# MahdiGhafoorian/NLML_HPE

Hardware: AMD Instinct MI355X
Metric: faces_per_sec (higher is better)
Workload: dtype f16x2s

## Files before the change

nlml_hpe_amd/csrc/abi.cpp:

```cpp
#include <hip/hip_runtime_api.h>

#include <cstdio>
#include <cstdlib>
#include <cstring>

#include "../../include/nlml_hpe.h"
#include "abi_internal.h"
#include "centroid_ref.h"
#include "layout.h"
#include "powell.h"

namespace nlml {
static thread_local char g_err[256] = "";
int fail(int code, const char* msg) {
  std::snprintf(g_err, sizeof g_err, "%s", msg ? msg : "unknown error");
  return code ? code : NLML_E_BADARG;
}
int hip_launch_status() {
  const hipError_t e = hipGetLastError();
  return e == hipSuccess ? 0 : fail((int)e, hipGetErrorString(e));
}
}

using namespace nlml;

static bool known_mode(int mode) { return mode == NLML_MODE_F32 || mode == NLML_MODE_BF16 || mode == NLML_MODE_F16X2 || mode == NLML_MODE_F16X2S; }
static bool split_f16(int mode) { return mode == NLML_MODE_F16X2 || mode == NLML_MODE_F16X2S; }

extern "C" {

int nlml_abi_version(void) { return NLML_ABI_VERSION; }
const char* nlml_last_error(void) { return g_err; }

int nlml_normalize_ipd(const float* raw, int64_t B, int normalize, float* out, uint8_t* valid, void* stream) {
  if (B < 0 || (B > 0 && (!raw || !out))) return fail(NLML_E_BADARG, "normalize_ipd: null buffer or negative B");
  if ((reinterpret_cast<uintptr_t>(raw) | reinterpret_cast<uintptr_t>(out)) & 15)
    return fail(NLML_E_BADARG, "normalize_ipd: raw/out must be 16-byte aligned");
  return launch_normalize_ipd(raw, B, normalize, out, valid, stream);
}

int nlml_normalize_centroid(const float* raw, int64_t B, float* out, uint8_t* valid, double* stats, void* stream) {
  if (B < 0 || (B > 0 && (!raw || !out))) return fail(NLML_E_BADARG, "normalize_centroid: null buffer or negative B");
  if ((reinterpret_cast<uintptr_t>(raw) | reinterpret_cast<uintptr_t>(out)) & 15)
    return fail(NLML_E_BADARG, "normalize_centroid: raw/out must be 16-byte aligned");
  if (reinterpret_cast<uintptr_t>(stats) & 7) return fail(NLML_E_BADARG, "normalize_centroid: stats must be 8-byte aligned");
  return launch_normalize_centroid(raw, B, out, valid, stats, stream);
}

int nlml_normalize_centroid_host(const float* h_raw, int64_t B, float* h_out, uint8_t* h_valid, double* h_stats) {
  if (B < 0 || (B > 0 && (!h_raw || !h_out))) return fail(NLML_E_BADARG, "normalize_centroid_host: null buffer or negative B");
  for (int64_t b = 0; b < B; ++b) {
    const int v = cn_face_host(h_raw + b * NLML_F_REFERENCE, h_out + b * NLML_F_REFERENCE, h_stats ? h_stats + 4 * b : nullptr);
    if (h_valid) h_valid[b] = (uint8_t)v;
  }
  return 0;
}

size_t nlml_encoder_heads_packed_bytes(int F, int mode) {
  if (F <= 0 || !known_mode(mode)) return 0;
  return blob_bytes_for(F, mode);
}

int nlml_encoder_heads_pack(int F, int mode, const float* const h_enc_w[6], const float* const h_enc_b[6],
                            const float* const h_head_w[3][5], const float* const h_head_b[3][5], void* h_blob,
                            size_t blob_bytes) {
  if (!known_mode(mode)) return fail(NLML_E_BADARG, "pack: unsupported mode");
  if (!h_enc_w || !h_enc_b || !h_head_w || !h_head_b) return fail(NLML_E_BADARG, "pack: null table");
  return pack_blob(F, mode, h_enc_w, h_enc_b, h_head_w, h_head_b, h_blob, blob_bytes);
}

static int check_blob_args(int64_t B, int F, const void* blob, size_t blob_bytes, const float* out, int* mode) {
  if (B < 0 || F <= 0) return fail(NLML_E_BADARG, "encoder_heads: negative B or bad F");
  if (B > 0 && (!blob || !out)) return fail(NLML_E_BADARG, "encoder_heads: null buffer");
  if (reinterpret_cast<uintptr_t>(blob) & 15) return fail(NLML_E_BADARG, "encoder_heads: blob must be 16-byte aligned");
  if (blob_bytes == blob_bytes_for(F, NLML_MODE_F32)) *mode = NLML_MODE_F32;
  else if (blob_bytes == blob_bytes_for(F, NLML_MODE_BF16)) *mode = NLML_MODE_BF16;
  else if (blob_bytes == blob_bytes_for(F, NLML_MODE_F16X2)) *mode = NLML_MODE_F16X2;
  else if (blob_bytes == blob_bytes_for(F, NLML_MODE_F16X2S)) *mode = NLML_MODE_F16X2S;
  else return fail(NLML_E_BADBLOB, "encoder_heads: blob size does not match F in any mode");
  return 0;
}

static const int64_t kSmallMax = 4096;
static int64_t streamed_min() {
  static const int64_t v = [] { const char* e = getenv("NLML_K2_STREAMED_MIN"); return e && e[0] ? (int64_t)atoll(e) : (int64_t)-1; }();
  return v;
}

enum K2Form { K2_FUSED, K2_SMALL, K2_STREAMED, K2_AUTO };

static int k2_forward(K2Form form, bool landmarks, const float* x, int64_t ldx, const float* raw, int normalize, int64_t B, int F,
                      const void* blob, size_t blob_bytes, float* out, float* latent, uint8_t* valid, void* workspace, size_t ws_bytes,
                      void* stream) {
  const char* no_input = nullptr;
  if (B > 0 && landmarks && !raw) no_input = "landmarks_to_pose: null raw";
  if (B > 0 && !landmarks && (!x || ldx < F)) no_input = "encoder_heads: null x or ldx < F";
  if (no_input && form == K2_AUTO && landmarks) return fail(NLML_E_BADARG, no_input);
  int mode = 0;
  if (int rc = check_blob_args(B, F, blob, blob_bytes, out, &mode)) return rc;
  if (form == K2_SMALL && !split_f16(mode)) return fail(NLML_E_BADARG, "small-batch path: NLML_MODE_F16X2 / NLML_MODE_F16X2S blob only");
  if (form == K2_STREAMED && mode != NLML_MODE_F16X2S) return fail(NLML_E_BADARG, "streamed-tail path: NLML_MODE_F16X2S blob only");
  if (no_input) return fail(NLML_E_BADARG, no_input);
  const int split = mode == NLML_MODE_F16X2S;
  if (form == K2_AUTO) {
    if (split_f16(mode) && B <= kSmallMax) form = K2_SMALL;
    else if (split && streamed_min() >= 0 && B >= streamed_min() && k2_input(x, ldx, raw, normalize, F).vec4) form = K2_STREAMED;
    else form = K2_FUSED;
  }
  if (form == K2_SMALL)
    return launch_encoder_heads_f16x2_small(x, ldx, raw, normalize, B, F, blob, out, latent, valid, workspace, ws_bytes, split, stream);
  if (form == K2_STREAMED)
    return launch_encoder_heads_f16x2_tailws(x, ldx, raw, normalize, B, F, blob, out, latent, valid, workspace, ws_bytes, stream);
  if (mode == NLML_MODE_BF16) return launch_encoder_heads_bf16(x, ldx, raw, normalize, B, F, blob, out, latent, valid, stream);
  if (split_f16(mode)) return launch_encoder_heads_f16x2(x, ldx, raw, normalize, B, F, blob, out, latent, valid, split, stream);
  return launch_encoder_heads_f32(x, ldx, raw, normalize, B, F, blob, out, latent, valid, nullptr, nullptr, stream);
}

int nlml_encoder_heads_fwd(const float* x, int64_t ldx, int64_t B, int F, const void* blob, size_t blob_bytes,
                           float* out, float* latent, uint8_t* valid, void* stream) {
  return k2_forward(K2_FUSED, false, x, ldx, nullptr, 0, B, F, blob, blob_bytes, out, latent, valid, nullptr, 0, stream);
}

int nlml_encoder_heads_fwd_debug(const float* x, int64_t ldx, int64_t B, int F, const void* blob, size_t blob_bytes,
                                 float* out, float* latent, float* pre_tanh, unsigned long long* stamps, void* stream) {
  int mode = 0;
  if (int rc = check_blob_args(B, F, blob, blob_bytes, out, &mode)) return rc;
  if (mode != NLML_MODE_F32) return fail(NLML_E_BADARG, "debug build: f32 blob only");
  if (B > 0 && (!x || ldx < F)) return fail(NLML_E_BADARG, "encoder_heads: null x or ldx < F");
  return launch_encoder_heads_f32(x, ldx, nullptr, 0, B, F, blob, out, latent, nullptr, pre_tanh, stamps, stream);
}

int nlml_landmarks_to_pose(const float* raw, int64_t B, int normalize, const void* blob, size_t blob_bytes,
                           float* out, float* latent, uint8_t* valid, void* stream) {
  return k2_forward(K2_FUSED, true, nullptr, 0, raw, normalize, B, NLML_F_REFERENCE, blob, blob_bytes, out, latent, valid, nullptr, 0, stream);
}

size_t nlml_encoder_heads_small_workspace_bytes(int64_t B, int F) { return small_workspace_bytes(B, F); }

int nlml_encoder_heads_fwd_small(const float* x, int64_t ldx, int64_t B, int F, const void* blob, size_t blob_bytes,
                                 float* out, float* latent, uint8_t* valid, void* workspace, size_t ws_bytes, void* stream) {
  return k2_forward(K2_SMALL, false, x, ldx, nullptr, 0, B, F, blob, blob_bytes, out, latent, valid, workspace, ws_bytes, stream);
}

int nlml_landmarks_to_pose_small(const float* raw, int64_t B, int normalize, const void* blob, size_t blob_bytes,
                                 float* out, float* latent, uint8_t* valid, void* workspace, size_t ws_bytes, void* stream) {
  return k2_forward(K2_SMALL, true, nullptr, 0, raw, normalize, B, NLML_F_REFERENCE, blob, blob_bytes, out, latent, valid, workspace, ws_bytes, stream);
}

int nlml_encoder_heads_fwd_streamed(const float* x, int64_t ldx, int64_t B, int F, const void* blob, size_t blob_bytes,
                                    float* out, float* latent, uint8_t* valid, void* workspace, size_t ws_bytes, void* stream) {
  return k2_forward(K2_STREAMED, false, x, ldx, nullptr, 0, B, F, blob, blob_bytes, out, latent, valid, workspace, ws_bytes, stream);
}

int nlml_landmarks_to_pose_streamed(const float* raw, int64_t B, int normalize, const void* blob, size_t blob_bytes,
                                    float* out, float* latent, uint8_t* valid, void* workspace, size_t ws_bytes, void* stream) {
  return k2_forward(K2_STREAMED, true, nullptr, 0, raw, normalize, B, NLML_F_REFERENCE, blob, blob_bytes, out, latent, valid, workspace, ws_bytes, stream);
}

size_t nlml_encoder_heads_workspace_bytes(int64_t B, int F) {
  const size_t a = small_workspace_bytes(B, F), b = tailws_workspace_bytes(B, F);
  return a > b ? a : b;
}

int nlml_encoder_heads_fwd_ws(const float* x, int64_t ldx, int64_t B, int F, const void* blob, size_t blob_bytes,
                              float* out, float* latent, uint8_t* valid, void* workspace, size_t ws_bytes, void* stream) {
  return k2_forward(K2_AUTO, false, x, ldx, nullptr, 0, B, F, blob, blob_bytes, out, latent, valid, workspace, ws_bytes, stream);
}

int nlml_landmarks_to_pose_ws(const float* raw, int64_t B, int normalize, const void* blob, size_t blob_bytes,
                              float* out, float* latent, uint8_t* valid, void* workspace, size_t ws_bytes, void* stream) {
  return k2_forward(K2_AUTO, true, nullptr, 0, raw, normalize, B, NLML_F_REFERENCE, blob, blob_bytes, out, latent, valid, workspace, ws_bytes, stream);
}

static int check_td_fast_alignment(const float* Wm, const float* x, int64_t ldx, const char* who) {
  if ((reinterpret_cast<uintptr_t>(Wm) & 15) || (reinterpret_cast<uintptr_t>(x) & 15) || (ldx & 3)) {
    static thread_local char msg[160];
    snprintf(msg, sizeof msg, "%s: NLML_TD_ORDER_FAST needs Wm and x 16-byte aligned and ldx %% 4 == 0", who);
    return fail(NLML_E_BADARG, msg);
  }
  return 0;
}

int nlml_tucker_objective_ex(const float* Wm, const float* x, int64_t ldx, const int32_t* x_index,
                             const double* params, const double* cos_params, int64_t N, double* err, double* x_hat,
                             int order, void* stream) {
  if (order != NLML_TD_ORDER_FAST && order != NLML_TD_ORDER_REFERENCE) return fail(NLML_E_BADARG, "tucker_objective: unknown order");
  if (N < 0) return fail(NLML_E_BADARG, "tucker_objective: negative N");
  if (N > 0 && (!Wm || !x || !params || !cos_params || !err)) return fail(NLML_E_BADARG, "tucker_objective: null buffer");
  if (N > 0 && ldx < NLML_F_REFERENCE) return fail(NLML_E_BADARG, "tucker_objective: ldx < 1404");
  if (N > 0 && order == NLML_TD_ORDER_FAST)
    if (int rc = check_td_fast_alignment(Wm, x, ldx, "tucker_objective")) return rc;
  return launch_tucker_objective(Wm, x, ldx, x_index, params, cos_params, N, err, x_hat, order, stream);
}

int nlml_tucker_objective(const float* Wm, const float* x, int64_t ldx, const int32_t* x_index,
                          const double* params, const double* cos_params, int64_t N, double* err, double* x_hat,
                          void* stream) {
  return nlml_tucker_objective_ex(Wm, x, ldx, x_index, params, cos_params, N, err, x_hat, NLML_TD_ORDER_REFERENCE, stream);
}

int nlml_video_post_ex(const float* pose_rad, const float* raw, const uint8_t* valid, int64_t S, double frame_w,
                       double frame_h, double alpha, double max_jump, double size, double* state, double* smoothed,
                       double* centre, double* endpoints, uint8_t* updated, void* stream) {
  if (S < 0) return fail(NLML_E_BADARG, "video_post: negative S");
  if (S > 0 && (!pose_rad || !raw || !state || !smoothed || !centre || !endpoints))
    return fail(NLML_E_BADARG, "video_post: null buffer");
  return launch_video_post(pose_rad, raw, valid, S, frame_w, frame_h, alpha, max_jump, size, state, smoothed, centre,
                           endpoints, updated, stream);
}

int nlml_video_post(const float* pose_rad, const float* raw, const uint8_t* valid, int64_t S, double frame_w,
                    double frame_h, double alpha, double max_jump, double size, double* state, double* smoothed,
                    double* centre, double* endpoints, void* stream) {
  return nlml_video_post_ex(pose_rad, raw, valid, S, frame_w, frame_h, alpha, max_jump, size, state, smoothed, centre, endpoints,
                            nullptr, stream);
}

int nlml_cosine_table(const float* angles_rad, int64_t n, const double* cos_params, int R, double* out, void* stream) {
  if (n < 0 || R < 0) return fail(NLML_E_BADARG, "cosine_table: negative size");
  if (n > 0 && R > 0 && (!angles_rad || !cos_params || !out)) return fail(NLML_E_BADARG, "cosine_table: null buffer");
  return launch_cosine_table(angles_rad, n, cos_params, R, out, stream);
}

int nlml_mode5_product(const float* core, const float* U_feat, int Q, int R5, int M, float* W, void* stream) {
  if (Q < 0 || R5 < 0 || M < 0) return fail(NLML_E_BADARG, "mode5_product: negative size");
  if (Q > 0 && M > 0 && (!W || (R5 > 0 && (!core || !U_feat)))) return fail(NLML_E_BADARG, "mode5_product: null buffer");
  return launch_mode5_product(core, U_feat, Q, R5, M, W, stream);
}

static bool eval_k_ok(int K) { return K >= 0 && K <= NLML_POSE_EVAL_MAX_INTERVALS; }
static int64_t eval_records(int64_t B) { return (B + NLML_POSE_EVAL_FACES_PER_RECORD - 1) / NLML_POSE_EVAL_FACES_PER_RECORD; }

size_t nlml_pose_eval_record_len(int n_intervals) { return eval_k_ok(n_intervals) ? (size_t)(12 + 2 * n_intervals) : 0; }
size_t nlml_pose_eval_result_len(int n_intervals) { return eval_k_ok(n_intervals) ? (size_t)(14 + 2 * n_intervals) : 0; }
size_t nlml_pose_eval_workspace_bytes(int64_t B, int n_intervals) {
  if (B < 0 || !eval_k_ok(n_intervals)) return 0;
  return (size_t)eval_records(B) * nlml_pose_eval_record_len(n_intervals) * sizeof(double);
}

static bool misaligned8(const void* p) { return (reinterpret_cast<uintptr_t>(p) & 7) != 0; }

int nlml_pose_eval(const float* pose_rad, const double* pred_deg, const uint8_t* valid, const double* gt_deg, int64_t B,
                   const double* h_lo, const double* h_hi, int decimals, const double* h_intervals, const int32_t* h_axes,
                   int n_intervals, void* workspace, size_t workspace_bytes, double* record_out, double* result_out,
                   double* pred_out, uint8_t* keep_out, void* stream) {
  if (B < 0) return fail(NLML_E_BADARG, "pose_eval: negative B");
  if ((pose_rad && pred_deg) || (B > 0 && !pose_rad && !pred_deg))
    return fail(NLML_E_BADARG, "pose_eval: give exactly one of pose_rad and pred_deg");
  if (B > 0 && !gt_deg) return fail(NLML_E_BADARG, "pose_eval: null gt_deg");
  if (!h_lo || !h_hi || !result_out) return fail(NLML_E_BADARG, "pose_eval: null lo / hi / result_out");
  if (!eval_k_ok(n_intervals)) return fail(NLML_E_BADARG, "pose_eval: number of intervals outside [0, NLML_POSE_EVAL_MAX_INTERVALS]");
  if (n_intervals > 0 && (!h_intervals || !h_axes)) return fail(NLML_E_BADARG, "pose_eval: null intervals / axes");
  if (decimals > 15) return fail(NLML_E_BADARG, "pose_eval: decimals > 15");
  const size_t need = nlml_pose_eval_workspace_bytes(B, n_intervals);
  if (workspace_bytes < need || (need > 0 && !workspace)) return fail(NLML_E_BADARG, "pose_eval: workspace too small");
  if (misaligned8(pred_deg) || misaligned8(gt_deg) || misaligned8(workspace) || misaligned8(record_out) || misaligned8(result_out) ||
      misaligned8(pred_out) || (reinterpret_cast<uintptr_t>(pose_rad) & 3))
    return fail(NLML_E_BADARG, "pose_eval: f64 buffers must be 8-byte aligned, pose_rad 4-byte aligned");
  PoseEvalArgs a{};
  for (int i = 0; i < 3; ++i) { a.lo[i] = h_lo[i]; a.hi[i] = h_hi[i]; }
  for (int k = 0; k < n_intervals; ++k) {
    if (h_axes[k] < 0 || h_axes[k] > 2) return fail(NLML_E_BADARG, "pose_eval: interval axis outside {0, 1, 2}");
    a.axes[k] = h_axes[k];
    a.ivl[k][0] = h_intervals[2 * k];
    a.ivl[k][1] = h_intervals[2 * k + 1];
  }
  a.scale = 1.0;
  for (int i = 0; i < decimals; ++i) a.scale *= 10.0;
  a.K = n_intervals;
  a.decimals = decimals;
  return launch_pose_eval(pose_rad, pred_deg, valid, gt_deg, B, a, static_cast<double*>(workspace), record_out, result_out, pred_out,
                          keep_out, stream);
}

int nlml_pose_eval_merge(const double* records, int64_t n, int n_intervals, double* record_out, double* result_out, void* stream) {
  if (n < 0) return fail(NLML_E_BADARG, "pose_eval_merge: negative record count");
  if (!eval_k_ok(n_intervals)) return fail(NLML_E_BADARG, "pose_eval_merge: number of intervals outside [0, NLML_POSE_EVAL_MAX_INTERVALS]");
  if ((n > 0 && !records) || !result_out) return fail(NLML_E_BADARG, "pose_eval_merge: null records / result_out");
  if (misaligned8(records) || misaligned8(record_out) || misaligned8(result_out))
    return fail(NLML_E_BADARG, "pose_eval_merge: buffers must be 8-byte aligned");
  return launch_pose_eval_merge(records, n, n_intervals, record_out, result_out, stream);
}

size_t nlml_powell_state_bytes(void) { return sizeof(PowellState); }

int nlml_powell_init(void* h_state, const double* h_x0, double xtol, double ftol) {
  if (!h_state || !h_x0) return fail(NLML_E_BADARG, "powell_init: null pointer");
  powell_init(*static_cast<PowellState*>(h_state), h_x0, xtol, ftol);
  return 0;
}

int nlml_powell_step(void* h_state, double fin, double* h_xeval) {
  if (!h_state || !h_xeval) return fail(NLML_E_BADARG, "powell_step: null pointer");
  PowellState& s = *static_cast<PowellState*>(h_state);
  const bool need = powell_step(s, fin);
  if (need) std::memcpy(h_xeval, s.xeval, sizeof s.xeval);
  return need ? 1 : 0;
}

int nlml_powell_result(const void* h_state, double* h_x, double* h_fval, int* h_nfev, int* h_nit, int* h_status) {
  if (!h_state || !h_x) return fail(NLML_E_BADARG, "powell_result: null pointer");
  const PowellState& s = *static_cast<const PowellState*>(h_state);
  std::memcpy(h_x, s.x, sizeof s.x);
  if (h_fval) *h_fval = s.fval;
  if (h_nfev) *h_nfev = s.nfev;
  if (h_nit) *h_nit = s.iter;
  if (h_status) *h_status = s.status;
  return 0;
}

int nlml_tucker_powell_ex(const float* Wm, const float* x, int64_t ldx, const double* cos_params, int64_t N,
                          const double* x0, double* result, double* fval, int32_t* nfev, int32_t* nit,
                          int32_t* status, int order, void* stream) {
  if (order != NLML_TD_ORDER_FAST && order != NLML_TD_ORDER_REFERENCE) return fail(NLML_E_BADARG, "tucker_powell: unknown order");
  if (N < 0) return fail(NLML_E_BADARG, "tucker_powell: negative N");
  if (N > 0 && (!Wm || !x || !cos_params || !result)) return fail(NLML_E_BADARG, "tucker_powell: null buffer");
  if (N > 0 && ldx < NLML_F_REFERENCE) return fail(NLML_E_BADARG, "tucker_powell: ldx < 1404");
  if (N > 0 && order == NLML_TD_ORDER_FAST)
    if (int rc = check_td_fast_alignment(Wm, x, ldx, "tucker_powell")) return rc;
  return launch_tucker_powell(Wm, x, ldx, cos_params, N, x0, result, fval, nfev, nit, status, order, stream);
}

int nlml_tucker_powell(const float* Wm, const float* x, int64_t ldx, const double* cos_params, int64_t N,
                       const double* x0, double* result, double* fval, int32_t* nfev, int32_t* nit,
                       int32_t* status, void* stream) {
  return nlml_tucker_powell_ex(Wm, x, ldx, cos_params, N, x0, result, fval, nfev, nit, status, NLML_TD_ORDER_REFERENCE, stream);
}

static_assert(PW_NMAX == 3 + NLML_TUCKER_RANK_MAX && PW_N == 3 + 5, "powell.h's state sizes follow the ranks");
static bool rank_ok(int r_id) { return r_id >= NLML_TUCKER_RANK_MIN && r_id <= NLML_TUCKER_RANK_MAX; }
static int bad_rank(const char* who, int r_id) {
  static thread_local char msg[160];
  snprintf(msg, sizeof msg, "%s: identity rank %d outside [%d, %d]", who, r_id, NLML_TUCKER_RANK_MIN, NLML_TUCKER_RANK_MAX);
  return fail(NLML_E_SHAPE, msg);
}

int nlml_tucker_objective_r(const float* Wm, const float* x, int64_t ldx, const int32_t* x_index, const double* params,
                            const double* cos_params, int64_t N, double* err, double* x_hat, int r_id, int order, void* stream) {
  if (!rank_ok(r_id)) return bad_rank("tucker_objective_r", r_id);
  if (r_id == 5) return nlml_tucker_objective_ex(Wm, x, ldx, x_index, params, cos_params, N, err, x_hat, order, stream);
  if (order != NLML_TD_ORDER_FAST && order != NLML_TD_ORDER_REFERENCE) return fail(NLML_E_BADARG, "tucker_objective_r: unknown order");
  if (N < 0) return fail(NLML_E_BADARG, "tucker_objective_r: negative N");
  if (N > 0 && (!Wm || !x || !params || !cos_params || !err)) return fail(NLML_E_BADARG, "tucker_objective_r: null buffer");
  if (N > 0 && ldx < NLML_F_REFERENCE) return fail(NLML_E_BADARG, "tucker_objective_r: ldx < 1404");
  if (N > 0 && order == NLML_TD_ORDER_FAST)
    if (int rc = check_td_fast_alignment(Wm, x, ldx, "tucker_objective_r")) return rc;
  return launch_tucker_objective_r(Wm, x, ldx, x_index, params, cos_params, N, err, x_hat, r_id, order, stream);
}

int nlml_tucker_powell_r(const float* Wm, const float* x, int64_t ldx, const double* cos_params, int64_t N, const double* x0,
                         double* result, double* fval, int32_t* nfev, int32_t* nit, int32_t* status, int r_id, int order,
                         void* stream) {
  if (!rank_ok(r_id)) return bad_rank("tucker_powell_r", r_id);
  if (r_id == 5) return nlml_tucker_powell_ex(Wm, x, ldx, cos_params, N, x0, result, fval, nfev, nit, status, order, stream);
  if (order != NLML_TD_ORDER_FAST && order != NLML_TD_ORDER_REFERENCE) return fail(NLML_E_BADARG, "tucker_powell_r: unknown order");
  if (N < 0) return fail(NLML_E_BADARG, "tucker_powell_r: negative N");
  if (N > 0 && (!Wm || !x || !cos_params || !result)) return fail(NLML_E_BADARG, "tucker_powell_r: null buffer");
  if (N > 0 && ldx < NLML_F_REFERENCE) return fail(NLML_E_BADARG, "tucker_powell_r: ldx < 1404");
  if (N > 0 && order == NLML_TD_ORDER_FAST)
    if (int rc = check_td_fast_alignment(Wm, x, ldx, "tucker_powell_r")) return rc;
  return launch_tucker_powell_r(Wm, x, ldx, cos_params, N, x0, result, fval, nfev, nit, status, r_id, order, stream);
}

static bool dim_ok(int n) { return n >= 3 + NLML_TUCKER_RANK_MIN && n <= 3 + NLML_TUCKER_RANK_MAX; }

size_t nlml_powell_state_bytes_n(int n) { return dim_ok(n) ? sizeof(PowellStateN) : 0; }

int nlml_powell_init_n(void* h_state, int n, const double* h_x0, double xtol, double ftol) {
  if (!dim_ok(n)) return bad_rank("powell_init_n", n - 3);
  if (!h_state || !h_x0) return fail(NLML_E_BADARG, "powell_init_n: null pointer");
  PowellStateN& s = *static_cast<PowellStateN*>(h_state);
  std::memset(h_state, 0, sizeof(PowellStateN));
  s.set_dim(n);
  powell_init(s, h_x0, xtol, ftol);
  return 0;
}

int nlml_powell_step_n(void* h_state, double fin, double* h_xeval) {
  if (!h_state || !h_xeval) return fail(NLML_E_BADARG, "powell_step_n: null pointer");
  PowellStateN& s = *static_cast<PowellStateN*>(h_state);
  if (!dim_ok(s.n)) return bad_rank("powell_step_n", s.n - 3);
  const bool need = powell_step(s, fin);
  if (need) std::memcpy(h_xeval, s.xeval, sizeof(double) * s.n);
  return need ? 1 : 0;
}

int nlml_powell_result_n(const void* h_state, double* h_x, double* h_fval, int* h_nfev, int* h_nit, int* h_status) {
  if (!h_state || !h_x) return fail(NLML_E_BADARG, "powell_result_n: null pointer");
  const PowellStateN& s = *static_cast<const PowellStateN*>(h_state);
  if (!dim_ok(s.n)) return bad_rank("powell_result_n", s.n - 3);
  std::memcpy(h_x, s.x, sizeof(double) * s.n);
  if (h_fval) *h_fval = s.fval;
  if (h_nfev) *h_nfev = s.nfev;
  if (h_nit) *h_nit = s.iter;
  if (h_status) *h_status = s.status;
  return 0;
}

}
```

nlml_hpe_amd/csrc/encoder_heads_f16x2_tailws.hip:

```cpp
#include <hip/hip_runtime.h>

#include "../../include/nlml_hpe.h"
#include "abi_internal.h"
#include "encoder_heads_f16x2_dev.h"
#include "layout.h"

#if defined(__HIP_DEVICE_COMPILE__) && !defined(__gfx950__)
#error "global_load_lds_dwordx4: gfx950"
#endif

namespace nlml {
namespace hx {

typedef unsigned u4 __attribute__((ext_vector_type(4)));
#ifdef TW_NO_PRIO
#define TW_PRIO(p) do { } while (0)
#else
#define TW_PRIO(p) __builtin_amdgcn_s_setprio(p)
#endif
typedef __attribute__((address_space(3))) const char LdsC;
typedef __attribute__((address_space(3))) char LdsW;

struct TwArgs {
  const void* blob;
  const u4* h3;
  float* out;
  float* latent;
  int64_t B, nfb;
};

constexpr int TW_SLOT = 65536;
constexpr int tw_bias_n16(int s) { return kStages[s].jobs * kStages[s].nb * 8; }
constexpr int tw_bias_off(int s) {
  int o = 0;
  for (int t = ST_E3; t < s; ++t) o += tw_bias_n16(t) * 16;
  return o;
}
constexpr int TW_O_BIAS = 2 * TW_SLOT;
constexpr int TW_O_LAT = TW_O_BIAS + ((tw_bias_off(NUM_STAGES) + 511) / 512) * 512;
constexpr int TW_LAT_WAVE = 3 * 2 * 256;
constexpr int TW_LDS = TW_O_LAT + 8 * TW_LAT_WAVE;
static_assert(TW_LDS <= 163840, "LDS map");

constexpr int TW_HEAD_UNITS = 9, TW_UNITS = 4 + 3 * TW_HEAD_UNITS;
__device__ __forceinline__ void tw_unit(const HdrRegs& H, int idx, uint32_t& off, uint32_t& n16) {
  constexpr uint32_t J3 = stage_job_w16_const(ST_E3), J4 = stage_job_w16_const(ST_E4), J5 = stage_job_w16_const(ST_E5);
  constexpr uint32_t K0 = stage_job_w16_const(ST_H0), K1 = stage_job_w16_const(ST_H1), K2 = stage_job_w16_const(ST_H2);
  constexpr uint32_t K3 = stage_job_w16_const(ST_H3), K4 = stage_job_w16_const(ST_H4);
  static_assert(2 * J3 * 16 == TW_SLOT && 2 * J4 * 16 <= TW_SLOT && J5 * 16 <= TW_SLOT && 4 * K0 * 16 <= TW_SLOT && K1 * 16 <= TW_SLOT &&
                    2 * K2 * 16 == TW_SLOT && 2 * K3 * 16 <= TW_SLOT && K4 * 16 <= TW_SLOT,
                "a unit fits a buffer");
  if (idx < 2) { n16 = 2 * J3; off = H.w_off(ST_E3) + idx * 2 * J3; }
  else if (idx == 2) { n16 = 2 * J4; off = H.w_off(ST_E4); }
  else if (idx == 3) { n16 = J5; off = H.w_off(ST_E5); }
  else {
    const int k = idx - 4, g = k / TW_HEAD_UNITS, r = k - TW_HEAD_UNITS * g;
    if (r == 0) { n16 = 4 * K0; off = H.w_off(ST_H0) + 4 * g * K0; }
    else if (r <= 4) { n16 = K1; off = H.w_off(ST_H1) + (4 * g + (r - 1)) * K1; }
    else if (r <= 6) { n16 = 2 * K2; off = H.w_off(ST_H2) + (4 * g + 2 * (r - 5)) * K2; }
    else if (r == 7) { n16 = 2 * K3; off = H.w_off(ST_H3) + 2 * g * K3; }
    else { n16 = K4; off = H.w_off(ST_H4) + g * K4; }
  }
}

template <int K16, int NCH = 2>
__device__ __forceinline__ void tw_job2(f32x16 (&acc)[2], LdsC* w0, LdsC* w1, int wstep, LdsC* b0, LdsC* b1, const h8 (&in)[K16][2]) {
  typedef const __attribute__((address_space(3))) h8 LdsH8;
#pragma unroll
  for (int c = 0; c < NCH; ++c)
#pragma unroll
    for (int q = 0; q < 4; ++q) {
      const f32x4 v = *reinterpret_cast<const __attribute__((address_space(3))) f32x4*>((c ? b1 : b0) + q * 16);
      acc[c][4 * q + 0] = v[0];
      acc[c][4 * q + 1] = v[1];
      acc[c][4 * q + 2] = v[2];
      acc[c][4 * q + 3] = v[3];
    }
  TW_PRIO(2);
#pragma unroll
  for (int ks = 0; ks < K16; ++ks) {
    h8 wf[NCH][2];
#pragma unroll
    for (int c = 0; c < NCH; ++c)
#pragma unroll
      for (int p = 0; p < 2; ++p) wf[c][p] = *reinterpret_cast<LdsH8*>((c ? w1 : w0) + ks * wstep + p * 1024);
#pragma unroll
    for (int t = 0; t < 3; ++t)
#pragma unroll
      for (int c = 0; c < NCH; ++c)
        acc[c] = __builtin_amdgcn_mfma_f32_32x32x16_f16(wf[c][t == 0 ? 1 : 0], in[ks][t == 1 ? 1 : 0], acc[c], 0, 0, 0);
  }
  TW_PRIO(0);
}

template <int K16>
__device__ __forceinline__ void tw_job2p(f32x16 (&acc)[2], LdsC* w0, LdsC* w1, int wstep, LdsC* b0, LdsC* b1, const h8 (&in)[K16][2]) {
  typedef const __attribute__((address_space(3))) h8 LdsH8;
#pragma unroll
  for (int c = 0; c < 2; ++c)
#pragma unroll
    for (int q = 0; q < 4; ++q) {
      const f32x4 v = *reinterpret_cast<const __attribute__((address_space(3))) f32x4*>((c ? b1 : b0) + q * 16);
      acc[c][4 * q + 0] = v[0];
      acc[c][4 * q + 1] = v[1];
      acc[c][4 * q + 2] = v[2];
      acc[c][4 * q + 3] = v[3];
    }
  h8 wf[2][2][2];
#pragma unroll
  for (int c = 0; c < 2; ++c)
#pragma unroll
    for (int p = 0; p < 2; ++p) wf[0][c][p] = *reinterpret_cast<LdsH8*>((c ? w1 : w0) + p * 1024);
  TW_PRIO(2);
  __builtin_amdgcn_sched_barrier(0);
#pragma unroll
  for (int ks = 0; ks < K16; ++ks) {
#pragma unroll
    for (int m = 0; m < 6; ++m) {
      const int t = m >> 1, c = m & 1;
      acc[c] = __builtin_amdgcn_mfma_f32_32x32x16_f16(wf[ks & 1][c][t == 0 ? 1 : 0], in[ks][t == 1 ? 1 : 0], acc[c], 0, 0, 0);
      __builtin_amdgcn_sched_barrier(0);
      if (m < 4 && ks + 1 < K16)
        wf[(ks + 1) & 1][m & 1][m < 2 ? 1 : 0] = *reinterpret_cast<LdsH8*>(((m & 1) ? w1 : w0) + (ks + 1) * wstep + (m < 2 ? 1024 : 0));
      __builtin_amdgcn_sched_barrier(0);
    }
  }
  TW_PRIO(0);
}

__global__ __launch_bounds__(512) void tail_ws_kernel(TwArgs a) {
  __shared__ __attribute__((aligned(1024))) char lds[TW_LDS];
  const int tid = threadIdx.x, lane = tid & 63, f = lane & 31, h = lane >> 5;
  const int wv = __builtin_amdgcn_readfirstlane(tid >> 6);
  const HdrRegs H = load_hdr(reinterpret_cast<const Header*>(a.blob));
  const h8* const blob8 = reinterpret_cast<const h8*>(a.blob);
  const f32x4* const blob4 = reinterpret_cast<const f32x4*>(a.blob);

  int64_t fbg = (int64_t)blockIdx.x * 8 + wv;
  const bool wave_live = fbg < a.nfb;
  fbg = wave_live ? fbg : a.nfb - 1;
  const int64_t row = fbg * 32 + f;
  const bool row_live = wave_live && row < a.B;

  LdsW* const ring = (LdsW*)(lds);
  auto issue = [&](int idx, int slot_off) {
    if (idx >= TW_UNITS) return;
    uint32_t off, n16;
    tw_unit(H, idx, off, n16);
    const int npieces = (int)(n16 >> 6);
#pragma unroll
    for (int i = 0; i < TW_SLOT / 8192; ++i) {
      const int pc = wv + 8 * i;
      if (pc < npieces)
        __builtin_amdgcn_global_load_lds((const __attribute__((address_space(1))) void*)(blob8 + off + pc * 64 + lane),
                                         (__attribute__((address_space(3))) void*)(ring + slot_off + pc * 1024), 16, 0, 0);
    }
  };
#ifdef TW_STAMPS
  int tw_u = 0;
#define TWS(i)                                                                                                                \
  do {                                                                                                                        \
    if (a.latent && lane == 0)                                                                                                \
      reinterpret_cast<unsigned long long*>(a.latent)[((size_t)blockIdx.x * 8 + wv) * 96 + (i)] = __builtin_amdgcn_s_memtime(); \
  } while (0)
#define TW_STAMP_MID() TWS(2 + 2 * tw_u)
#define TW_STAMP_END() do { TWS(3 + 2 * tw_u); ++tw_u; } while (0)
#else
#define TWS(i) do { } while (0)
#define TW_STAMP_MID() do { } while (0)
#define TW_STAMP_END() do { } while (0)
#endif
  TWS(0);
  issue(0, 0);

  {
    f32x4* const bl = reinterpret_cast<f32x4*>(lds + TW_O_BIAS);
#pragma unroll
    for (int s = ST_E3; s < NUM_STAGES; ++s) {
      const f32x4* src = blob4 + H.b_off(s);
      for (int i = tid; i < tw_bias_n16(s); i += 512) bl[tw_bias_off(s) / 16 + i] = src[i];
    }
  }
  h8 x3[16][2];
  {
    const u4* src = a.h3 + (size_t)fbg * (16 * 2 * 64) + lane;
#pragma unroll
    for (int ks = 0; ks < 16; ++ks)
#pragma unroll
      for (int p = 0; p < 2; ++p) x3[ks][p] = __builtin_bit_cast(h8, src[(ks * 2 + p) * 64]);
  }
  asm volatile("s_waitcnt vmcnt(0)" ::: "memory");
  __syncthreads();
  TWS(1);

  int cur = 0;
  LdsC* const bias0 = (LdsC*)(lds + TW_O_BIAS) + 64 * h;
  LdsC* const wl0 = (LdsC*)(lds) + lane * 16;
  LdsW* const latw = (LdsW*)(lds + TW_O_LAT) + wv * TW_LAT_WAVE + f * 8;
#ifdef TW_NO_SKEW
  const bool late = false;
#else
  const bool late = wv >= 4;
#endif
#define TW_BEGIN(idx) issue((idx) + 1, cur ^ TW_SLOT); LdsC* const wl = wl0 + cur
#define TW_MID()                                      \
  TW_STAMP_MID();                                     \
  asm volatile("s_waitcnt vmcnt(0)" ::: "memory");    \
  if (late) __syncthreads()
#define TW_END()                                      \
  asm volatile("s_waitcnt vmcnt(0)" ::: "memory");    \
  if (!late) __syncthreads();                         \
  TW_STAMP_END();                                     \
  cur ^= TW_SLOT

  f32x16 acc[2];
  auto emit = [&](auto act, const f32x16& ac, float inv, h8 (&d0)[2], h8 (&d1)[2]) {
    h8 fr[2][2];
    frags_from_acc<decltype(act)::value>(ac, inv, fr);
    d0[0] = fr[0][0]; d0[1] = fr[0][1]; d1[0] = fr[1][0]; d1[1] = fr[1][1];
  };
  constexpr std::integral_constant<int, ACT_RELU> RELU{};
  constexpr std::integral_constant<int, ACT_TANH> TANH{};
  const float inv3 = H.inv_scale[ST_E3], inv4 = H.inv_scale[ST_E4], inv5 = H.inv_scale[ST_E5];
  constexpr int JB3 = (int)(stage_job_w16_const(ST_E3) * 16), JB4 = (int)(stage_job_w16_const(ST_E4) * 16);

  h8 x4[8][2];
#pragma unroll
  for (int u = 0; u < 2; ++u) {
    TW_BEGIN(u);
    LdsC* const b = bias0 + tw_bias_off(ST_E3) + (2 * u) * 128;
    tw_job2p<16>(acc, wl, wl + JB3, 2048, b, b + 128, x3);
    TW_MID();
    emit(RELU, acc[0], inv3, x4[4 * u], x4[4 * u + 1]);
    emit(RELU, acc[1], inv3, x4[4 * u + 2], x4[4 * u + 3]);
    TW_END();
  }
  h8 x5[4][2];
  {
    TW_BEGIN(2);
    LdsC* const b = bias0 + tw_bias_off(ST_E4);
    tw_job2<8>(acc, wl, wl + JB4, 2048, b, b + 128, x4);
    TW_MID();
    emit(TANH, acc[0], inv4, x5[0], x5[1]);
    emit(TANH, acc[1], inv4, x5[2], x5[3]);
    TW_END();
  }
  {
    TW_BEGIN(3);
    LdsC* const b = bias0 + tw_bias_off(ST_E5);
    tw_job2<4>(acc, wl, wl + 2048, 4096, b, b + 128, x5);
    TW_MID();
#ifndef TW_STAMPS
    if (a.latent && row_live) {
#pragma unroll
      for (int nb = 0; nb < 2; ++nb)
#pragma unroll
        for (int q = 0; q < 16; ++q) {
          const int rowi = 32 * nb + (q & 3) + 8 * (q >> 2) + 4 * h, g = rowi >> 4, cc = rowi & 15;
          if (g < 3 && cc < 3) a.latent[row * NLML_LATENT + 3 * g + cc] = acc[nb][q] * inv5;
        }
    }
#endif
#pragma unroll
    for (int nb = 0; nb < 2; ++nb) {
      h8 fr[2][2];
      frags_from_acc<ACT_NONE>(acc[nb], inv5, fr);
#pragma unroll
      for (int p = 0; p < 2; ++p)
#pragma unroll
        for (int pc = 0; pc < 2; ++pc)
          if (2 * nb + p < 3 && h == 0) {
            const u4 t = __builtin_bit_cast(u4, fr[p][pc]);
            typedef unsigned u2 __attribute__((ext_vector_type(2)));
            *reinterpret_cast<__attribute__((address_space(3))) u2*>(latw + ((2 * nb + p) * 2 + pc) * 256) = u2{t[0], t[1]};
          }
    }
    TW_END();
  }
#pragma unroll 1
  for (int g = 0; g < 3; ++g) {
    const int u0 = 4 + TW_HEAD_UNITS * g;
    const float i0 = H.inv_scale[ST_H0], i1 = H.inv_scale[ST_H1], i2 = H.inv_scale[ST_H2], i3 = H.inv_scale[ST_H3];
    h8 xa[8][2];
    {
      TW_BEGIN(u0);
      h8 xin[1][2];
#pragma unroll
      for (int pc = 0; pc < 2; ++pc) {
        typedef unsigned u2 __attribute__((ext_vector_type(2)));
        const u2 t = *reinterpret_cast<const __attribute__((address_space(3))) u2*>((LdsC*)latw + (g * 2 + pc) * 256);
        xin[0][pc] = __builtin_bit_cast(h8, u4{h == 0 ? t[0] : 0u, h == 0 ? t[1] : 0u, 0u, 0u});
      }
      LdsC* const b = bias0 + tw_bias_off(ST_H0) + (4 * g) * 128;
      constexpr int JB = (int)(stage_job_w16_const(ST_H0) * 16);
#pragma unroll
      for (int jj = 0; jj < 2; ++jj) {
        tw_job2<1>(acc, wl + (2 * jj) * JB, wl + (2 * jj + 1) * JB, 2048, b + (2 * jj) * 128, b + (2 * jj + 1) * 128, xin);
        if (jj == 1) { TW_MID(); }
        emit(RELU, acc[0], i0, xa[4 * jj], xa[4 * jj + 1]);
        emit(RELU, acc[1], i0, xa[4 * jj + 2], xa[4 * jj + 3]);
      }
      TW_END();
    }
    h8 xb[16][2];
#pragma unroll
    for (int j = 0; j < 4; ++j) {
      TW_BEGIN(u0 + 1 + j);
      LdsC* const b = bias0 + tw_bias_off(ST_H1) + (4 * g + j) * 256;
      tw_job2p<8>(acc, wl, wl + 2048, 4096, b, b + 128, xa);
      TW_MID();
      emit(RELU, acc[0], i1, xb[4 * j], xb[4 * j + 1]);
      emit(RELU, acc[1], i1, xb[4 * j + 2], xb[4 * j + 3]);
      TW_END();
    }
    h8 xc[8][2];
#pragma unroll
    for (int u = 0; u < 2; ++u) {
      TW_BEGIN(u0 + 5 + u);
      constexpr int JB = (int)(stage_job_w16_const(ST_H2) * 16);
      LdsC* const b = bias0 + tw_bias_off(ST_H2) + (4 * g + 2 * u) * 128;
      tw_job2p<16>(acc, wl, wl + JB, 2048, b, b + 128, xb);
      TW_MID();
      emit(RELU, acc[0], i2, xc[4 * u], xc[4 * u + 1]);
      emit(RELU, acc[1], i2, xc[4 * u + 2], xc[4 * u + 3]);
      TW_END();
    }
    h8 xd[4][2];
    {
      TW_BEGIN(u0 + 7);
      LdsC* const b = bias0 + tw_bias_off(ST_H3) + (2 * g) * 128;
      tw_job2p<8>(acc, wl, wl + (int)(stage_job_w16_const(ST_H3) * 16), 2048, b, b + 128, xc);
      TW_MID();
      emit(RELU, acc[0], i3, xd[0], xd[1]);
      emit(RELU, acc[1], i3, xd[2], xd[3]);
      TW_END();
    }
    {
      TW_BEGIN(u0 + 8);
      LdsC* const b = bias0 + tw_bias_off(ST_H4) + g * 128;
      tw_job2<4, 1>(acc, wl, wl, 2048, b, b, xd);
      TW_MID();
      if (h == 0 && row_live) a.out[row * 3 + g] = acc[0][0] * H.inv_scale[ST_H4];
      TW_END();
    }
  }
#undef TW_BEGIN
#undef TW_MID
#undef TW_END
}

}

int launch_tail_ws(const void* blob, const void* h3, int64_t nfb, int64_t B, float* out, float* latent, void* stream) {
  if (B == 0) return 0;
  hx::TwArgs a;
  a.blob = blob; a.h3 = reinterpret_cast<const hx::u4*>(h3); a.out = out; a.latent = latent; a.B = B; a.nfb = nfb;
  hipLaunchKernelGGL(hx::tail_ws_kernel, dim3((unsigned)((nfb + 7) / 8)), dim3(512), 0, reinterpret_cast<hipStream_t>(stream), a);
  return hip_launch_status();
}

}
```

Before: 79.07 million.

## Stream h3 input loads into first E3 job and route fused calls to tailws path

The streamed-tail kernel now loads only the first few k-slices of the h3 activations before the prologue barrier and fetches the remaining slices inside the first E3 MFMA loop, a fixed distance ahead. This overlaps global input latency with matrix work instead of stalling on all 32 loads up front. Separately, the fused entry point can hand over to the streamed kernel with a stream-ordered workspace allocation when an env threshold is set. The env parsing is also hardened, and the streamed path now stays disabled by default. The in-loop loads add vmcnt pressure and may interact with the waitcnt at the mid barrier.

```diff
diff --git a/nlml_hpe_amd/csrc/abi.cpp b/nlml_hpe_amd/csrc/abi.cpp
--- a/nlml_hpe_amd/csrc/abi.cpp
+++ b/nlml_hpe_amd/csrc/abi.cpp
@@ -1,5 +1,6 @@
 #include <hip/hip_runtime_api.h>
 
+#include <cerrno>
 #include <cstdio>
 #include <cstdlib>
 #include <cstring>
@@ -82,9 +83,30 @@
 }
 
 static const int64_t kSmallMax = 4096;
+static const int64_t kStreamedNever = INT64_MAX;
 static int64_t streamed_min() {
-  static const int64_t v = [] { const char* e = getenv("NLML_K2_STREAMED_MIN"); return e && e[0] ? (int64_t)atoll(e) : (int64_t)-1; }();
+  static const int64_t v = [] {
+    const char* e = getenv("NLML_K2_STREAMED_MIN");
+    if (!e || !e[0]) return kStreamedNever;
+    char* end = nullptr;
+    errno = 0;
+    const long long n = strtoll(e, &end, 10);
+    if (end == e || *end != '\0' || errno == ERANGE || n <= kSmallMax) return kStreamedNever;
+    return (int64_t)n;
+  }();
   return v;
+}
+static bool streamed_pays(int mode, int64_t B, const float* x, int64_t ldx, const float* raw, int normalize, int F) {
+  return mode == NLML_MODE_F16X2S && B >= streamed_min() && k2_input(x, ldx, raw, normalize, F).vec4;
+}
+
+static bool handover_alloc(size_t bytes, hipStream_t st, void** ws) {
+  hipStreamCaptureStatus cap = hipStreamCaptureStatusNone;
+  if (hipStreamIsCapturing(st, &cap) == hipSuccess && cap == hipStreamCaptureStatusNone && hipMallocAsync(ws, bytes, st) == hipSuccess && *ws)
+    return true;
+  (void)hipGetLastError();
+  *ws = nullptr;
+  return false;
 }
 
 enum K2Form { K2_FUSED, K2_SMALL, K2_STREAMED, K2_AUTO };
@@ -104,8 +126,17 @@
   const int split = mode == NLML_MODE_F16X2S;
   if (form == K2_AUTO) {
     if (split_f16(mode) && B <= kSmallMax) form = K2_SMALL;
-    else if (split && streamed_min() >= 0 && B >= streamed_min() && k2_input(x, ldx, raw, normalize, F).vec4) form = K2_STREAMED;
+    else if (streamed_pays(mode, B, x, ldx, raw, normalize, F)) form = K2_STREAMED;
     else form = K2_FUSED;
+  } else if (form == K2_FUSED && !workspace && B > 0 && streamed_pays(mode, B, x, ldx, raw, normalize, F)) {
+    hipStream_t st = reinterpret_cast<hipStream_t>(stream);
+    const size_t bytes = tailws_workspace_bytes(B, F);
+    void* ws = nullptr;
+    if (handover_alloc(bytes, st, &ws)) {
+      const int rc = launch_encoder_heads_f16x2_tailws(x, ldx, raw, normalize, B, F, blob, out, latent, valid, ws, bytes, stream);
+      if (hipFreeAsync(ws, st) != hipSuccess) (void)hipGetLastError();
+      return rc;
+    }
   }
   if (form == K2_SMALL)
     return launch_encoder_heads_f16x2_small(x, ldx, raw, normalize, B, F, blob, out, latent, valid, workspace, ws_bytes, split, stream);
diff --git a/nlml_hpe_amd/csrc/encoder_heads_f16x2_tailws.hip b/nlml_hpe_amd/csrc/encoder_heads_f16x2_tailws.hip
--- a/nlml_hpe_amd/csrc/encoder_heads_f16x2_tailws.hip
+++ b/nlml_hpe_amd/csrc/encoder_heads_f16x2_tailws.hip
@@ -1,4 +1,6 @@
 #include <hip/hip_runtime.h>
+
+#include <type_traits>
 
 #include "../../include/nlml_hpe.h"
 #include "abi_internal.h"
@@ -30,6 +32,10 @@
 };
 
 constexpr int TW_SLOT = 65536;
+#ifndef TW_H3_AHEAD
+#define TW_H3_AHEAD 4
+#endif
+static_assert(TW_H3_AHEAD >= 1 && TW_H3_AHEAD <= 16, "TW_H3_AHEAD");
 constexpr int tw_bias_n16(int s) { return kStages[s].jobs * kStages[s].nb * 8; }
 constexpr int tw_bias_off(int s) {
   int o = 0;
@@ -93,8 +99,9 @@
   TW_PRIO(0);
 }
 
-template <int K16>
-__device__ __forceinline__ void tw_job2p(f32x16 (&acc)[2], LdsC* w0, LdsC* w1, int wstep, LdsC* b0, LdsC* b1, const h8 (&in)[K16][2]) {
+template <int K16, int AHEAD = 0>
+__device__ __forceinline__ void tw_job2p(f32x16 (&acc)[2], LdsC* w0, LdsC* w1, int wstep, LdsC* b0, LdsC* b1,
+                                         std::conditional_t<(AHEAD > 0), h8, const h8> (&in)[K16][2], const u4* src = nullptr) {
   typedef const __attribute__((address_space(3))) h8 LdsH8;
 #pragma unroll
   for (int c = 0; c < 2; ++c)
@@ -122,6 +129,8 @@
       __builtin_amdgcn_sched_barrier(0);
       if (m < 4 && ks + 1 < K16)
         wf[(ks + 1) & 1][m & 1][m < 2 ? 1 : 0] = *reinterpret_cast<LdsH8*>(((m & 1) ? w1 : w0) + (ks + 1) * wstep + (m < 2 ? 1024 : 0));
+      if constexpr (AHEAD > 0)
+        if (m >= 4 && ks + AHEAD < K16) in[ks + AHEAD][m - 4] = __builtin_bit_cast(h8, src[((ks + AHEAD) * 2 + (m - 4)) * 64]);
       __builtin_amdgcn_sched_barrier(0);
     }
   }
@@ -171,6 +180,12 @@
 #define TW_STAMP_END() do { } while (0)
 #endif
   TWS(0);
+  h8 x3[16][2];
+  const u4* const x3src = a.h3 + (size_t)fbg * (16 * 2 * 64) + lane;
+#pragma unroll
+  for (int ks = 0; ks < TW_H3_AHEAD; ++ks)
+#pragma unroll
+    for (int p = 0; p < 2; ++p) x3[ks][p] = __builtin_bit_cast(h8, x3src[(ks * 2 + p) * 64]);
   issue(0, 0);
 
   {
@@ -180,14 +195,6 @@
       const f32x4* src = blob4 + H.b_off(s);
       for (int i = tid; i < tw_bias_n16(s); i += 512) bl[tw_bias_off(s) / 16 + i] = src[i];
     }
-  }
-  h8 x3[16][2];
-  {
-    const u4* src = a.h3 + (size_t)fbg * (16 * 2 * 64) + lane;
-#pragma unroll
-    for (int ks = 0; ks < 16; ++ks)
-#pragma unroll
-      for (int p = 0; p < 2; ++p) x3[ks][p] = __builtin_bit_cast(h8, src[(ks * 2 + p) * 64]);
   }
   asm volatile("s_waitcnt vmcnt(0)" ::: "memory");
   __syncthreads();
@@ -229,7 +236,8 @@
   for (int u = 0; u < 2; ++u) {
     TW_BEGIN(u);
     LdsC* const b = bias0 + tw_bias_off(ST_E3) + (2 * u) * 128;
-    tw_job2p<16>(acc, wl, wl + JB3, 2048, b, b + 128, x3);
+    if (u == 0) tw_job2p<16, TW_H3_AHEAD>(acc, wl, wl + JB3, 2048, b, b + 128, x3, x3src);
+    else tw_job2p<16>(acc, wl, wl + JB3, 2048, b, b + 128, x3);
     TW_MID();
     emit(RELU, acc[0], inv3, x4[4 * u], x4[4 * u + 1]);
     emit(RELU, acc[1], inv3, x4[4 * u + 2], x4[4 * u + 3]);
```

Result: no change. 78.95 million, median of 2 (-0.2%).
